# TheJacksonLaboratory/cnn_autoencoder

Hardware: AMD Instinct MI355X
Metric: tiles/sec, compress+decompress round trip of 1024x1024x3 histology tiles (higher is better)
Workload: dtype f32 (f16x3 split MFMA: 3 f16 MFMAs per product, fp32 accumulate)

## Files before the change

### cnn_autoencoder_amd/csrc/cae_api.hip

```cpp
#include "cae_hip.h"
#include "cae_internal.hpp"
#include "cae_kernels.hpp"
#include "cae_kernels_f16.hpp"
#include "cae_launch.hpp"
#include "cae_pack.hpp"

#include <algorithm>
#include <cmath>
#include <cstdio>
#include <cstdlib>
#include <cstring>
#include <string>

namespace cae {

thread_local std::string g_last_error;
thread_local int64_t g_last_ticket = 0;
thread_local int g_force_fp32 = 0;

int fail(int code, const char *fmt, ...) {
    char buf[512];
    va_list ap;
    va_start(ap, fmt);
    vsnprintf(buf, sizeof buf, fmt, ap);
// ... 198 lines not shown

static int pick_slot(int a, int b) {
    for (int k = 1; k <= 3; ++k)
        if (k != a && k != b) return k;
    return 1;
}

static bool stages_need_fp32(const Layer &l) {
    if (round_ct(l.cin) <= 4) return false;
    for (const Layer::Stage &sg : l.stages)
        if (sg.gdn || sg.add_res || sg.post_act) return true;
    return false;
}

static int run_stages(Model *m, const Layer &l, bool synthesis, int n, int ch, int cw, const float *&cur, int &cur_idx,
                      int &cur_planes, hipStream_t st, bool f16 = false, int *flag = nullptr) {
    if (f16 && stages_need_fp32(l)) {
        const int tmp = pick_slot(cur_idx, cur_idx);
        const size_t rows = (size_t)n * cur_planes * ch;
        if (synthesis)
            hipLaunchKernelGGL(c8s_to_c8_kernel<true>, dim3(ew_grid(rows * cw)), dim3(256), 0, st, (const char *)cur,
                               (float *)m->ws[tmp].p, rows, cw);
        else
            hipLaunchKernelGGL(c8s_to_c8_kernel<false>, dim3(ew_grid(rows * cw)), dim3(256), 0, st, (const char *)cur,
                               (float *)m->ws[tmp].p, rows, cw);
        HIP_TRY(hipGetLastError());
        cur = (const float *)m->ws[tmp].p;
        cur_idx = tmp;
        int rc = run_stages(m, l, synthesis, n, ch, cw, cur, cur_idx, cur_planes, st, false, nullptr);
        if (rc) return rc;
        const int back = pick_slot(cur_idx, cur_idx);
        const size_t orows = (size_t)n * cur_planes * ch;
        if (synthesis)
            hipLaunchKernelGGL(c8_to_c8s_kernel<true>, dim3(ew_grid(orows * cw)), dim3(256), 0, st, cur, (char *)m->ws[back].p,
                               orows, cw, flag);
        else
            hipLaunchKernelGGL(c8_to_c8s_kernel<false>, dim3(ew_grid(orows * cw)), dim3(256), 0, st, cur, (char *)m->ws[back].p,
                               orows, cw, flag);
        HIP_TRY(hipGetLastError());
        cur = (const float *)m->ws[back].p;
        cur_idx = back;
        return CAE_OK;
    }
    const float *unit_in = cur;
    const int unit_idx = cur_idx, unit_planes = cur_planes;
    for (const Layer::Stage &sg : l.stages) {
        const int ctin = round_ct(l.cin);
        const int out_idx = pick_slot(unit_idx, cur_idx);
        LayerArgs b = layer_args(m, cur, cur_planes, m->ws[out_idx].p, n, ch, cw, ch, cw, ctin, l.cin, OUT_C8, sg.act,
                                 f16 ? flag : nullptr);
        b.bias = sg.bias.get<float>();
        b.beta = sg.beta.get<float>();
        b.res = sg.add_res ? unit_in : nullptr;
        b.res_planes = unit_planes;
        b.post_act = sg.post_act;
        int rc;
        if (f16) {
            if (!sg.wp16 || (sg.gdn && !sg.gp16)) return fail(CAE_ERR_ARG, "stage uploaded before precision 1 was selected");
            b.wp = sg.wp16.get<float>();
            b.gp = sg.gp16.get<float>();
            rc = launch_conv_s1_f16(m->ks, ctin, synthesis, sg.gdn, l.cin, b, st);
// ... 244 lines not shown
}

static int analysis_impl(cae_model_t *mm, const void *tiles, int fmt, int n, int h, int w, void *latents, bool symbols,
                         float *const *levels, void *stream) {
    Model *m = reinterpret_cast<Model *>(mm);
    if (!m || !tiles || !latents) return fail(CAE_ERR_ARG, "NULL argument");
    if (symbols && m->ent.channels == 0) return fail(CAE_ERR_ARG, "entropy model not set");
    if (n < 1 || h < 2 || w < 2) return fail(CAE_ERR_ARG, "bad tile batch %dx%dx%d", n, h, w);
    if (fmt != CAE_FMT_U8_HWC && fmt != CAE_FMT_F32_NCHW) return fail(CAE_ERR_ARG, "bad pixel format %d", fmt);
    for (auto &l : m->enc)
        if (!l.set) return fail(CAE_ERR_ARG, "analysis layer not set");
    int rc;
    if ((rc = check_reflect_levels(m, h, w))) return rc;
    hipStream_t st = (hipStream_t)stream;
    std::lock_guard<std::mutex> lk(m->mu);
    if ((rc = m->ensure_device()) || (rc = m->order_stream(stream))) return rc;
    const bool f16 = m->f16_usable();
    const bool first_fused = f16 ? (bool)m->enc[0].wp_edge16 : (bool)m->enc[0].wp_edge;
    int64_t ticket = 0;
    g_last_ticket = 0;
    int *flag = f16 ? m->next_flag(&ticket) : m->flags_dev;

    const int p0 = f16 ? 2 * ((m->c_org + 15) / 16) : (m->c_org + 7) / 8;
    auto row_bytes = [&](int cw) { return f16 ? c8s_row_bytes<false>(cw) : (size_t)cw * 32; };
    size_t in_bytes = first_fused ? 0 : (size_t)n * p0 * h * row_bytes(w);
    size_t maxact = 0;
    {
        int ch = h, cw = w;
        for (int i = 0; i < m->L; ++i) {
            if (!m->enc[i].stages.empty())
                maxact = std::max(maxact, (size_t)n * round_ct(m->enc[i].cin) * 4 * ch * row_bytes(cw));
            ch = (ch + 1) / 2;
            cw = (cw + 1) / 2;
            if (i + 1 < m->L) maxact = std::max(maxact, (size_t)n * m->enc[i].ct * 4 * ch * row_bytes(cw));
        }
    }
    const bool u8_wide = f16 && !first_fused && fmt == CAE_FMT_U8_HWC;
    if (u8_wide) maxact = std::max(maxact, (size_t)n * p0 * h * w * 32);
    bool need_third_slot = false;
    for (auto &l : m->enc)
        need_third_slot |= l.stages.size() > 1 || (f16 && (!conv_f16_fits(m->ks, l.ct, l.gdn) || stages_need_fp32(l)));
    if ((rc = m->ensure_ws(0, in_bytes))) return rc;
    if (maxact && ((rc = m->ensure_ws(1, maxact)) || (rc = m->ensure_ws(2, maxact)))) return rc;
    if (maxact && need_third_slot && (rc = m->ensure_ws(3, maxact))) return rc;

    ProfScope prof(m, CAE_ANALYSIS, st);
    prof.begin();
    if (!first_fused) {
        const size_t tot = (size_t)n * p0 * h * w;
        if (f16) {
            if (fmt == CAE_FMT_U8_HWC) {
                hipLaunchKernelGGL(u8hwc_to_c8_kernel, dim3(ew_grid(tot)), dim3(256), 0, st, (const uint8_t *)tiles,
                                   (float *)m->ws[1].p, n, h, w, m->c_org, p0);
                hipLaunchKernelGGL(c8_to_c8s_kernel<false>, dim3(ew_grid(tot)), dim3(256), 0, st, (const float *)m->ws[1].p,
                                   (char *)m->ws[0].p, (size_t)n * p0 * h, w, flag);
            } else {
                hipLaunchKernelGGL(nchw_to_c8s_kernel<false>, dim3(ew_grid(tot)), dim3(256), 0, st,
                                   (const float *)tiles, (char *)m->ws[0].p, n, m->c_org, h, w, p0, flag);
            }
        } else if (fmt == CAE_FMT_U8_HWC) {
            hipLaunchKernelGGL(u8hwc_to_c8_kernel, dim3(ew_grid(tot)), dim3(256), 0, st, (const uint8_t *)tiles,
                               (float *)m->ws[0].p, n, h, w, m->c_org, p0);
        } else {
            hipLaunchKernelGGL(nchw_to_c8_kernel, dim3(ew_grid(tot)), dim3(256), 0, st, (const float *)tiles,
                               (float *)m->ws[0].p, n, m->c_org, h * w, p0);
        }
        HIP_TRY(hipGetLastError());
    }
    prof.end();

    const float *cur = (const float *)m->ws[0].p;
    int cur_planes = p0, ch = h, cw = w;
    int cur_idx = 0;
    for (int i = 0; i < m->L; ++i) {
        const Layer &l = m->enc[i];
        const bool last = i == m->L - 1;
        if (!l.stages.empty() && (rc = run_stages(m, l, false, n, ch, cw, cur, cur_idx, cur_planes, st, f16, flag))) return rc;
        const int out_idx = pick_slot(cur_idx, cur_idx);
        LayerArgs a = layer_args(m, cur, cur_planes, last ? latents : m->ws[out_idx].p, n, ch, cw, (ch + 1) / 2, (cw + 1) / 2,
                                 l.ct, l.cout, last ? (symbols ? OUT_SYM : OUT_NCHW) : OUT_C8, l.act, flag);
        a.wp = l.wp.get<float>();
        a.bias = l.bias.get<float>();
        a.gp = l.gp.get<float>();
        a.beta = l.beta.get<float>();
        if (last && symbols) a.medians = m->medians_dev.get<float>();
        prof.begin();
        if (i == 0 && first_fused) {
            FirstArgs f{tiles, fmt == CAE_FMT_U8_HWC ? 1 : 0, l.cin};
            if (f16) {
                a.wp = l.wp_edge16.get<float>();
                a.gp = l.gp16.get<float>();
                if ((rc = launch_first_f16(m->ks, l.ct, l.gdn, a, f, st))) return rc;
            } else {
                a.wp = l.wp_edge.get<float>();
                if ((rc = launch_first(m->ks, l.ct, l.gdn, a, f, st))) return rc;
            }
        } else if (f16 && conv_f16_fits(m->ks, l.ct, l.gdn) && !(l.gdn && l.ct > 4 && last)) {
            a.wp = l.wp16.get<float>();
            a.gp = l.gp16.get<float>();
            if ((rc = launch_conv_f16(m->ks, l.ct, l.gdn, l.cin, a, st))) return rc;
        } else if (f16) {
            const int tmp_in = pick_slot(cur_idx, out_idx);
            const size_t rows = (size_t)n * cur_planes * ch;
            hipLaunchKernelGGL(c8s_to_c8_kernel<false>, dim3(ew_grid(rows * cw)), dim3(256), 0, st, (const char *)cur,
                               (float *)m->ws[tmp_in].p, rows, cw);
            HIP_TRY(hipGetLastError());
            a.in = (const float *)m->ws[tmp_in].p;
            void *final_out = a.out;
            if (!last) a.out = m->ws[cur_idx == 0 ? pick_slot(tmp_in, out_idx) : cur_idx].p;
            if ((rc = launch_conv(m->ks, l.ct, l.gdn, l.cin, a, st))) return rc;
            if (!last) {
                const size_t orows = (size_t)n * l.ct * 4 * a.OH;
                hipLaunchKernelGGL(c8_to_c8s_kernel<false>, dim3(ew_grid(orows * a.OW)), dim3(256), 0, st, (const float *)a.out,
                                   (char *)final_out, orows, a.OW, flag);
                HIP_TRY(hipGetLastError());
                a.out = final_out;
            }
        } else {
            if ((rc = launch_conv(m->ks, l.ct, l.gdn, l.cin, a, st))) return rc;
        }
        prof.end();
        if (!last && levels && levels[i]) {
            const size_t t2 = (size_t)n * l.cout * a.OH * a.OW;
            if (f16)
                hipLaunchKernelGGL(c8s_to_nchw_kernel<false>, dim3(ew_grid(t2)), dim3(256), 0, st, (const char *)a.out,
                                   levels[i], n, l.cout, a.OH, a.OW, l.ct * 4);
            else
                hipLaunchKernelGGL(c8_to_nchw_kernel, dim3(ew_grid(t2)), dim3(256), 0, st, (const float *)a.out,
                                   levels[i], n, l.cout, a.OH * a.OW, l.ct * 4);
            HIP_TRY(hipGetLastError());
        }
        cur = (const float *)a.out;
        cur_planes = l.ct * 4;
        ch = a.OH;
        cw = a.OW;
        cur_idx = out_idx;
    }
    return CAE_OK;
}

static int synthesis_impl(cae_model_t *mm, const float *latents, const int32_t *symbols, int n, int lh, int lw, void *out,
                          int fmt, float *const *bridges, float *const *colors, void *stream, int scale = 0);

int cae_synthesis(cae_model_t *mm, const float *latents, int n, int lh, int lw, void *out, int fmt,
                  float *const *bridges, void *stream) {
    if (!latents) return fail(CAE_ERR_ARG, "NULL argument");
    return synthesis_impl(mm, latents, nullptr, n, lh, lw, out, fmt, bridges, nullptr, stream);
}
// ... 504 lines not shown
```

### cnn_autoencoder_amd/csrc/cae_kernels.hpp

```cpp
#pragma once
#include <hip/hip_runtime.h>
#include <stdint.h>
#include <type_traits>
#include <utility>

namespace cae {

typedef float f32x16 __attribute__((ext_vector_type(16)));
typedef float f32x4 __attribute__((ext_vector_type(4)));

enum OutFmt { OUT_C8 = 0, OUT_NCHW = 1, OUT_U8HWC = 2, OUT_SYM = 3, OUT_PMAP = 4 };

struct LayerArgs {
    const float *in;
    void *out;
    const float *wp;
    const float *bias;
    const float *gp;
    const float *beta;
    const float *zero;
    int N, H, W, OH, OW;
    int in_planes;
    int cci;
    int out_planes;
    int cout;
    int tiles_x, tiles_y;
    int outfmt;
// ... 2 lines not shown
    int res_planes;
    int post_act;
    const float *medians;
    const void *pm;
    int *flag;
};

__device__ __forceinline__ uint8_t clip_u8(float q) {
    return (uint8_t)__builtin_fmaxf(__builtin_fminf(q, 255.0f), 0.0f);
}
__device__ __forceinline__ int round_sym(float d) {
    return (int)rintf(__builtin_fminf(__builtin_fmaxf(d, -1073741824.0f), 1073741824.0f));
}

template <int N, class F, int... I>
__device__ __forceinline__ void static_for_impl(F &&f, std::integer_sequence<int, I...>) {
    (f(std::integral_constant<int, I>{}), ...);
}
template <int N, class F>
__device__ __forceinline__ void static_for(F &&f) {
    static_for_impl<N>(static_cast<F &&>(f), std::make_integer_sequence<int, N>{});
}

__device__ __forceinline__ int reflect_idx(int i, int n) {
    i = i < 0 ? -i : i;
    i = i >= n ? 2 * n - 2 - i : i;
    i = i < 0 ? 0 : i;
    return i >= n ? n - 1 : i;
}

__device__ __forceinline__ void glds16(const void *gsrc, void *lds_wave_base) {
    __builtin_amdgcn_global_load_lds((const __attribute__((address_space(1))) void *)gsrc,
                                     (__attribute__((address_space(3))) void *)lds_wave_base, 16, 0, 0);
}

__device__ __forceinline__ void wait_vm0() { asm volatile("s_waitcnt vmcnt(0)" ::: "memory"); }

__device__ __forceinline__ constexpr int acc_row(int r) { return (r & 3) + 8 * (r >> 2); }

__device__ __forceinline__ void load_acc_tile(f32x16 &a, const float *vec, int ct, int h) {
#pragma unroll
    for (int g = 0; g < 4; ++g) {
        const f32x4 v = *(const f32x4 *)(vec + 32 * ct + 8 * g + 4 * h);
#pragma unroll
        for (int k = 0; k < 4; ++k) a[4 * g + k] = v[k];
    }
}

template <int CT>
__device__ __forceinline__ void init_acc(f32x16 (&acc)[CT], const float *vec, int h, float fill) {
#pragma unroll
    for (int ct = 0; ct < CT; ++ct) {
        if (vec) {
// ... 1146 lines not shown
```

### cnn_autoencoder_amd/csrc/cae_kernels_f16.hpp

```cpp
#pragma once
#include "cae_kernels.hpp"

namespace cae {

constexpr int F16_ISSUERS = 2;
#define ISSUER(w, NW, NI) ((w) < (NI) ? (w) : -1)

typedef _Float16 f16x8 __attribute__((ext_vector_type(8)));
typedef _Float16 f16x4 __attribute__((ext_vector_type(4)));


__device__ __forceinline__ void split_f16(float v, _Float16 &hi, _Float16 &lo) {
    hi = (_Float16)v;
    lo = (_Float16)(v - (float)hi);
}

typedef unsigned u32x2v __attribute__((ext_vector_type(2)));
__device__ __forceinline__ u32x2v split2_f16(float a, float b) {
    typedef float f32x2 __attribute__((ext_vector_type(2)));
    typedef _Float16 f16x2 __attribute__((ext_vector_type(2)));
    const f32x2 ab = {a, b};
    const unsigned hi = __builtin_bit_cast(unsigned, __builtin_convertvector(ab, f16x2));
    float l0, l1;
    asm("v_fma_mix_f32 %0, %1, -1.0, %2 op_sel_hi:[1,0,0]" : "=v"(l0) : "v"(hi), "v"(a));
// ... 97 lines not shown
                const f16x8 gh = *(const f16x8 *)(gb + ((co * 2 + s) * 2 + 0) * 1024);
                const f16x8 gl = *(const f16x8 *)(gb + ((co * 2 + s) * 2 + 1) * 1024);
#pragma unroll
                for (int pt = 0; pt < PT; ++pt) nrm[pt][co] = mfma3(gh, gl, sh[pt], sl[pt], nrm[pt][co]);
            }
        }
        ++sc;
    }
#pragma unroll
    for (int pt = 0; pt < PT; ++pt) {
#pragma unroll
        for (int ct = 0; ct < CT; ++ct)
#pragma unroll
            for (int r = 0; r < 16; ++r) {
                const float nv = nrm[pt][ct][r];
                if constexpr (INVERSE)
                    y[PT0 + pt][ct][r] *= __builtin_amdgcn_sqrtf(nv) * pisc[pt];
                else
                    y[PT0 + pt][ct][r] *= __builtin_amdgcn_rsqf(nv);
            }
    }
}

template <bool SP>
__host__ __device__ __forceinline__ size_t c8s_row_bytes(int w) {
    return SP ? (size_t)((w + 63) >> 6) * 2048 : (size_t)((w + 31) >> 5) * 1024;
}
template <bool SP>
__host__ __device__ __forceinline__ unsigned c8s_piece(int x) {
    return SP ? (unsigned)(x >> 6) * 2048u + (unsigned)(x & 1) * 1024u + (unsigned)((x & 63) >> 1) * 16u
              : (unsigned)(x >> 5) * 1024u + (unsigned)(x & 31) * 16u;
}

template <int CT, bool SP = false>
__device__ __forceinline__ void store_split_f16(const f32x16 (&acc)[CT], const LayerArgs &p, int n, int oy, int ox, int h,
                                                int ct0 = 0) {
    {
        char *out = (char *)p.out;
        float mx = 0.0f;
#pragma unroll
        for (int ct = 0; ct < CT; ++ct)
#pragma unroll
            for (int r = 0; r < 16; r += 2)
                mx = absmax3(mx, acc[ct][r], acc[ct][r + 1]);
        raise_if_over(mx, p.flag);
        const size_t row_bytes = c8s_row_bytes<SP>(p.OW), plane_bytes = (size_t)p.OH * row_bytes;
        char *dst0 = out + (((size_t)n * p.out_planes + 4 * ct0) * p.OH + oy) * row_bytes + c8s_piece<SP>(ox) + 512 * h;
#pragma unroll
        for (int ct = 0; ct < CT; ++ct)
#pragma unroll
            for (int g = 0; g < 4; ++g) {
                typedef unsigned u32x2 __attribute__((ext_vector_type(2)));
                typedef unsigned u32x4 __attribute__((ext_vector_type(4)));
                u32x2 yh, xl;
                { const u32x2v t_ = split2_f16(acc[ct][4 * g + 0], acc[ct][4 * g + 1]); yh[0] = t_[0]; xl[0] = t_[1]; }
// ... 34 lines not shown

template <int CT, bool SP = false, int EPI = 0>
__device__ __forceinline__ void store_tiles_f16(f32x16 (&acc)[CT], const LayerArgs &p, int n, int oy, int ox,
                                                int h, bool valid) {
    if (!valid) return;
    if (p.outfmt == OUT_C8) {
        if constexpr (EPI & 1) {
            const float slope = p.act == 0 ? 1.0f : (p.act == 1 ? 0.01f : 0.0f);
#pragma unroll
            for (int ct = 0; ct < CT; ++ct)
#pragma unroll
                for (int r = 0; r < 16; ++r) acc[ct][r] = acc[ct][r] > 0.0f ? acc[ct][r] : slope * acc[ct][r];
        }
        if constexpr (EPI & 2) {
            if (p.res) add_residual_f16<CT, SP>(acc, p, n, oy, ox, h);
        }
        store_split_f16<CT, SP>(acc, p, n, oy, ox, h);
    } else {
        store_tiles<CT, false>(acc, p, n, oy, ox, h, valid);
    }
}

constexpr int CONV_F16_NW = 8;
template <int KS, int CT, bool GDN, int S = 2, bool SP = false, bool ZP = false, bool RES = false>
__global__ void __launch_bounds__(CONV_F16_NW * 64, 1) conv_s2_f16_kernel(const LayerArgs p) {
    constexpr int NW = CONV_F16_NW, PT = 8 / NW;
    constexpr int PAD = KS / 2;
    constexpr int TX = 16, TY = 16;
    constexpr int WH = S * TX + KS - S;
    constexpr int PLANE_PIECES = TY * WH;
    constexpr int HALO_PIECES = 4 * PLANE_PIECES;
    constexpr int HALO_INSTR = (HALO_PIECES + 63) / 64;
    constexpr int W_INSTR = KS * CT * 2;
    constexpr int W_BYTES = W_INSTR * 1024;
    constexpr int G_BYTES = GDN ? CT * 4096 : 0;
    constexpr int CONV_STAGE = W_BYTES + HALO_INSTR * 1024;
    constexpr int STAGE_BYTES = CONV_STAGE > G_BYTES ? CONV_STAGE : G_BYTES;
    constexpr int NI = NW / F16_ISSUERS > 0 ? NW / F16_ISSUERS : 1;
    constexpr int MAXP = (HALO_INSTR + NI - 1) / NI;
    extern __shared__ __attribute__((aligned(16))) char smem[];

    const int lane = threadIdx.x & 63;
    const int wave = __builtin_amdgcn_readfirstlane(threadIdx.x >> 6);
    const int h = lane >> 5, m = lane & 31;

    int bid = xcd_tile_order(blockIdx.x, gridDim.x);
    const int tx = bid % p.tiles_x;
    bid /= p.tiles_x;
    const int ty = bid % p.tiles_y;
    const int n = bid / p.tiles_y;
    const int oy0 = ty * TY, ox0 = tx * TX;

    const size_t plane_bytes = (size_t)p.H * c8s_row_bytes<SP>(p.W);
    const char *in_n = (const char *)p.in + (size_t)n * p.in_planes * plane_bytes;
    unsigned hoff[MAXP][KS];
#pragma unroll
    for (int i = 0; i < MAXP; ++i) {
        int pc = (ISSUER(wave, NW, NI) + i * NI) * 64 + lane;
        pc = pc < HALO_PIECES ? pc : HALO_PIECES - 1;
        const int plhl = pc / PLANE_PIECES;
        const int rem = pc - plhl * PLANE_PIECES;
        const int r = rem / WH, x = rem - r * WH;
        const int xi = S * ox0 - PAD + x;
// ... 430 lines not shown
                const int t0 = 4 * s + half, t1 = 4 * s + 2 + half;
                const int o0 = t0 < KS * KS ? ((t0 / KS) * WH + (t0 % KS)) * 16 : -1;
                const int o1 = t1 < KS * KS ? ((t1 / KS) * WH + (t1 % KS)) * 16 : -1;
                f32x4 v0 = {0.f, 0.f, 0.f, 0.f}, v1 = {0.f, 0.f, 0.f, 0.f};
                if (o0 >= 0) v0 = *(const f32x4 *)(hb + o0);
                if (o1 >= 0) v1 = *(const f32x4 *)(hb + o1);
                const f32x4 v = h ? v1 : v0;
                { const u32x2v t_ = split2_f16(v[0], v[1]); bhw[2 * half] = t_[0]; blw[2 * half] = t_[1]; }
                { const u32x2v t_ = split2_f16(v[2], v[3]); bhw[2 * half + 1] = t_[0]; blw[2 * half + 1] = t_[1]; }
            }
            const f16x8 bh = __builtin_bit_cast(f16x8, bhw), bl = __builtin_bit_cast(f16x8, blw);
#pragma unroll
            for (int ct = 0; ct < CT; ++ct) {
                const f16x8 ah = *(const f16x8 *)(wb + ((s * CT + ct) * 2 + 0) * 1024);
                const f16x8 al = *(const f16x8 *)(wb + ((s * CT + ct) * 2 + 1) * 1024);
                acc[ct] = mfma3(ah, al, bh, bl, acc[ct]);
            }
        }
        __builtin_amdgcn_wave_barrier();
        if (has_next) commit();
        __builtin_amdgcn_wave_barrier();
        if constexpr (GDN) gdn_resident_pipe_f16<CT, false>(acc, gbuf, beta_lds, lane);
        const int oy = ty * TY + 2 * wave + (m >> 4), ox = tx * TX + (m & 15);
        store_tiles_f16<CT, false, !GDN>(acc, p, n, oy, ox, h, oy < p.OH && ox < p.OW);
    }
    if constexpr (!U8)
        if (bad) *p.flag = 1;
}

__host__ __device__ __forceinline__ size_t pmap_record(int n, int OH, int OW, int oy, int ox) {
    return ((((size_t)n * OH + oy) * 2 + (ox & 1)) * (OW >> 1) + (ox >> 1)) * 32;
}

template <int CT, int LDS_JT>
__device__ __forceinline__ void store_pmap_f16(const f32x16 (&y)[CT], const LayerArgs &p, char *tbuf, int n, int oy, int par,
                                               int j0, int lane, bool row_valid, const char *pm_lds) {
    const int h = lane >> 5, m = lane & 31;
    f32x16 pm;
#pragma unroll
    for (int r = 0; r < 16; ++r) pm[r] = 0.0f;
    float mx = 0.0f;
#pragma unroll
    for (int jt = 0; jt < CT; ++jt)
#pragma unroll
        for (int s = 0; s < 2; ++s) {
            const char *ab = (jt < LDS_JT ? pm_lds : (const char *)p.pm) + lane * 16;
            u32x4v hw, lw;
// ... 574 lines not shown
```

### cnn_autoencoder_amd/csrc/cae_launch.hpp

```cpp
#pragma once
#include <hip/hip_runtime.h>

#include <map>
#include <mutex>
#include <utility>

#include "cae_hip.h"
#include "cae_internal.hpp"

#define HIP_TRY(expr)                                                                             \
    do {                                                                                          \
        hipError_t e_ = (expr);                                                                   \
        if (e_ != hipSuccess) return ::cae::fail(CAE_ERR_HIP, "%s: %s", #expr, hipGetErrorString(e_));  \
    } while (0)

#define CAE_TRY(expr)                          \
    do {                                       \
        const int rc_ = (expr);                \
        if (rc_ != CAE_OK) return rc_;         \
    } while (0)

namespace cae {
inline std::mutex &launch_mutex() {
    static std::mutex mu;
// ... 17 lines not shown
    int dev = 0;
    HIP_TRY(hipGetDevice(&dev));
    static std::map<int, int> known;
    std::lock_guard<std::mutex> lock(launch_mutex());
    auto it = known.find(dev);
    if (it == known.end()) {
        int n = 0;
        HIP_TRY(hipDeviceGetAttribute(&n, hipDeviceAttributeMultiprocessorCount, dev));
        it = known.emplace(dev, n).first;
    }
    cus = it->second;
    return CAE_OK;
}

template <class Args>
Args with_launch_facts(const Args &a, int w, int h, int tx, int ty, int cci) {
    Args b = a;
    b.tiles_x = (w + tx - 1) / tx;
    b.tiles_y = (h + ty - 1) / ty;
    b.cci = cci;
    return b;
}

struct LayerArgs;
struct FirstArgs;
int launch_conv(int ks, int ct, bool gdn, int cin, const LayerArgs &a, hipStream_t st);
int launch_conv_s1(int ks, int ct, bool zeropad, bool gdn, int cin, const LayerArgs &a, hipStream_t st);
int launch_deconv(int ks, int ct, bool gdn, int cin, const LayerArgs &a, hipStream_t st);
int launch_gdn(int ct, bool inverse, const LayerArgs &a, hipStream_t st);
int launch_first(int ks, int ct, bool gdn, const LayerArgs &a, const FirstArgs &f, hipStream_t st);
int launch_last(int ks, int cin, const LayerArgs &a, hipStream_t st);
int launch_conv_f16(int ks, int ct, bool gdn, int cin, const LayerArgs &a, hipStream_t st);
int launch_deconv_f16(int ks, int ct, bool gdn, int cin, const LayerArgs &a, hipStream_t st);
int launch_conv_s1_f16(int ks, int ct, bool synthesis, bool gdn, int cin, const LayerArgs &a, hipStream_t st);
int launch_color_f16(int ks, int cin, const LayerArgs &a, hipStream_t st);
bool conv_f16_fits(int ks, int ct, bool gdn);
bool last_f16_fits(int ks, int cin);
int launch_color_small(int ks, bool split, const void *in, int in_planes, int cin, const float *w, const float *bias,
                       int n, int h, int w_px, int cout, void *out, int outfmt, int *flag, hipStream_t st);
int launch_nchw_to_u8hwc(const float *in, void *out, int n, int c, size_t hw, hipStream_t st);
int launch_first_f16(int ks, int ct, bool gdn, const LayerArgs &a, const FirstArgs &f, hipStream_t st);
int launch_last_f16(int ks, int cin, const LayerArgs &a, hipStream_t st);
int launch_gdn_f16(int ct, bool inverse, const LayerArgs &a, hipStream_t st);
}
```

### cnn_autoencoder_amd/csrc/cae_launch_conv_f16.hip

```cpp
#include "cae_hip.h"
#include "cae_internal.hpp"
#include "cae_launch.hpp"
#include "cae_kernels_f16.hpp"
namespace cae {
constexpr int LDS_LIMIT = 160 * 1024;

constexpr int conv_f16_lds(int ks, int ct, bool gdn, int wh) {
    const int halo_instr = (4 * 16 * wh + 63) / 64;
    const int conv_stage = ks * ct * 2 * 1024 + halo_instr * 1024;
    const int g_bytes = gdn ? ct * 4096 : 0;
    return 2 * (conv_stage > g_bytes ? conv_stage : g_bytes);
}
constexpr int conv_f16_halo_width(int ks, int stride) { return stride * 16 + ks - stride; }

bool conv_f16_fits(int ks, int ct, bool gdn) {
    if (gdn && ct > 4) gdn = false;
    return conv_f16_lds(ks, ct, gdn, conv_f16_halo_width(ks, 2)) <= LDS_LIMIT;
}

static LayerArgs conv_f16_facts(const LayerArgs &a, int cin) {
    return with_launch_facts(a, a.OW, a.OH, 16, 16, (cin + 15) / 16);
}

template <int KS, int CT, bool GDN>
static int launch_conv_f16_t(int cin, const LayerArgs &args, hipStream_t st) {
    constexpr int NW = CONV_F16_NW;
    constexpr int LDS = conv_f16_lds(KS, CT, GDN, conv_f16_halo_width(KS, 2));
    if constexpr (LDS > LDS_LIMIT) {
        return fail(CAE_ERR_UNSUPPORTED, "f16x3: this kernel_size/channel combination exceeds the LDS; use fp32");
    } else {
        auto kern = conv_s2_f16_kernel<KS, CT, GDN>;
        CAE_TRY(ensure_lds((const void *)kern, LDS));
        const LayerArgs a = conv_f16_facts(args, cin);
        const unsigned grid = (unsigned)((size_t)a.N * a.tiles_x * a.tiles_y);
        hipLaunchKernelGGL(kern, dim3(grid), dim3(NW * 64), LDS, st, a);
        HIP_TRY(hipGetLastError());
        return CAE_OK;
    }
}

#define DISPATCH_F16(FN, KS_)                                                               \
    switch (ct) {                                                                          \
        case 1: return gdn ? FN<KS_, 1, true>(cin, a, st) : FN<KS_, 1, false>(cin, a, st); \
        case 2: return gdn ? FN<KS_, 2, true>(cin, a, st) : FN<KS_, 2, false>(cin, a, st); \
        case 4: return gdn ? FN<KS_, 4, true>(cin, a, st) : FN<KS_, 4, false>(cin, a, st); \
        case 6: {  \
            const int rc6 = FN<KS_, 6, false>(cin, a, st);                                 \
            return rc6 || !gdn ? rc6 : launch_gdn_f16(6, false, a, st);                    \
        }                                                                                  \
        default: return fail(CAE_ERR_UNSUPPORTED, "unsupported channel tiles %d", ct);      \
    }

template <int KS, int CT, bool GDN, bool SYN, bool ZP>
static int launch_conv_s1_f16_t(int cin, const LayerArgs &args, hipStream_t st) {
    constexpr int NW = CONV_F16_NW;
    constexpr int LDS = conv_f16_lds(KS, CT, GDN, conv_f16_halo_width(KS, 1));
    if constexpr (LDS > LDS_LIMIT) {
        return fail(CAE_ERR_UNSUPPORTED, "f16x3: this kernel_size/channel combination exceeds the LDS; use fp32");
    } else {
        auto kern = conv_s2_f16_kernel<KS, CT, GDN, 1, SYN, ZP, (CT <= 4)>;
        CAE_TRY(ensure_lds((const void *)kern, LDS));
        const LayerArgs a = conv_f16_facts(args, cin);
        const unsigned grid = (unsigned)((size_t)a.N * a.tiles_x * a.tiles_y);
        hipLaunchKernelGGL(kern, dim3(grid), dim3(NW * 64), LDS, st, a);
        HIP_TRY(hipGetLastError());
        return CAE_OK;
    }
}

int launch_conv_s1_f16(int ks, int ct, bool synthesis, bool gdn, int cin, const LayerArgs &a, hipStream_t st) {
    if ((gdn || a.res || a.post_act) && ct > 4)
        return fail(CAE_ERR_UNSUPPORTED, "f16x3: GDN / residual stages wider than 128 channels run on the fp32 path");
#define S1_SIDE(KS_, CT_, GDN_) \
    return synthesis ? launch_conv_s1_f16_t<KS_, CT_, GDN_, true, true>(cin, a, st) \
                     : launch_conv_s1_f16_t<KS_, CT_, GDN_, false, false>(cin, a, st)
#define S1_CASE(KS_)                                                                   \
    switch (ct) {                                                                      \
        case 1: if (gdn) { S1_SIDE(KS_, 1, true); } else { S1_SIDE(KS_, 1, false); }   \
        case 2: if (gdn) { S1_SIDE(KS_, 2, true); } else { S1_SIDE(KS_, 2, false); }   \
        case 4: if (gdn) { S1_SIDE(KS_, 4, true); } else { S1_SIDE(KS_, 4, false); }   \
        case 6: S1_SIDE(KS_, 6, false);                                                \
        default: return fail(CAE_ERR_UNSUPPORTED, "unsupported channel tiles %d", ct);  \
    }
    if (ks == 3) { S1_CASE(3) }
    if (ks == 5) { S1_CASE(5) }
#undef S1_CASE
#undef S1_SIDE
    return fail(CAE_ERR_UNSUPPORTED, "kernel_size %d not supported (3 or 5)", ks);
}

int launch_color_f16(int ks, int cin, const LayerArgs &a, hipStream_t st) {
    if (ks == 3) return launch_conv_s1_f16_t<3, 1, false, true, false>(cin, a, st);
    if (ks == 5) return launch_conv_s1_f16_t<5, 1, false, true, false>(cin, a, st);
    return fail(CAE_ERR_UNSUPPORTED, "kernel_size %d not supported (3 or 5)", ks);
}

int launch_conv_f16(int ks, int ct, bool gdn, int cin, const LayerArgs &a, hipStream_t st) {
    if (ks == 3) { DISPATCH_F16(launch_conv_f16_t, 3) }
// ... 6 lines not shown
```

### cnn_autoencoder_amd/csrc/cae_launch_edge_f16.hip

```cpp
#include <algorithm>

#include "cae_hip.h"
#include "cae_internal.hpp"
#include "cae_launch.hpp"
#include "cae_kernels_f16.hpp"
namespace cae {
template <int KS, int CT, bool GDN>
static int launch_first_f16_t(const LayerArgs &a, const FirstArgs &f, hipStream_t st) {
    using G = FirstGeomF16<KS, CT, GDN>;
    constexpr int LDS = G::LDS_BYTES;
    if constexpr (LDS > 160 * 1024) {
        return fail(CAE_ERR_UNSUPPORTED, "f16x3: first-layer operands exceed the LDS for this shape; use fp32");
    } else {
        auto kern_u8 = conv_first_f16_kernel<KS, CT, GDN, true>;
        auto kern_f32 = conv_first_f16_kernel<KS, CT, GDN, false>;
        int n_cu = 0;
        CAE_TRY(ensure_lds((const void *)kern_u8, LDS));
        CAE_TRY(ensure_lds((const void *)kern_f32, LDS));
        CAE_TRY(device_cus(n_cu));
        const LayerArgs b = with_launch_facts(a, a.OW, a.OH, G::TX, G::TY, (f.cin + 7) / 8);
        const size_t total = (size_t)b.N * b.tiles_x * b.tiles_y;
        if (total > 0x7fffffff) return fail(CAE_ERR_ARG, "batch too large");
        const unsigned grid = (unsigned)std::min<size_t>(total, (size_t)std::max(n_cu, 1));
        hipLaunchKernelGGL(f.in_is_u8 ? kern_u8 : kern_f32, dim3(grid), dim3(G::NW * 64), LDS, st, b, f);
// ... 3 lines not shown
}

int launch_first_f16(int ks, int ct, bool gdn, const LayerArgs &a, const FirstArgs &f, hipStream_t st) {
#define FIRST_F16(KS_)                                                                                       \
    switch (ct) {                                                                                            \
        case 1: return gdn ? launch_first_f16_t<KS_, 1, true>(a, f, st) : launch_first_f16_t<KS_, 1, false>(a, f, st); \
        case 2: return gdn ? launch_first_f16_t<KS_, 2, true>(a, f, st) : launch_first_f16_t<KS_, 2, false>(a, f, st); \
        case 4: return gdn ? launch_first_f16_t<KS_, 4, true>(a, f, st) : launch_first_f16_t<KS_, 4, false>(a, f, st); \
        case 6: {                                                                                            \
            const int rc6 = launch_first_f16_t<KS_, 6, false>(a, f, st);                                     \
            return rc6 || !gdn ? rc6 : launch_gdn_f16(6, false, a, st);                                      \
        }                                                                                                    \
        default: return fail(CAE_ERR_UNSUPPORTED, "unsupported channel tiles %d", ct);                       \
    }
    if (ks == 3) { FIRST_F16(3) }
    if (ks == 5) { FIRST_F16(5) }
    return fail(CAE_ERR_UNSUPPORTED, "kernel_size %d not supported (3 or 5)", ks);
}

template <int CT, bool INVERSE>
static int launch_gdn_f16_t(const LayerArgs &a, hipStream_t st) {
    constexpr int LDS = CT * CT * 4096 + CT * 32 * 4;
    static_assert(LDS <= 160 * 1024, "packed gamma must fit the LDS");
    auto kern = gdn_f16_kernel<CT, INVERSE, INVERSE>;
    int n_cu = 0;
    CAE_TRY(ensure_lds((const void *)kern, LDS));
    CAE_TRY(device_cus(n_cu));
    const size_t groups = c8s_row_bytes<INVERSE>(a.OW) / 1024;
    const size_t total = (size_t)a.N * a.OH * groups;
    if (total > 0x7fffffff) return fail(CAE_ERR_ARG, "batch too large");
    const unsigned grid = (unsigned)std::min<size_t>((total + 3) / 4, (size_t)std::max(n_cu, 1));
    hipLaunchKernelGGL(kern, dim3(grid), dim3(256), LDS, st, a);
    HIP_TRY(hipGetLastError());
    return CAE_OK;
}

int launch_gdn_f16(int ct, bool inverse, const LayerArgs &a, hipStream_t st) {
    if (a.outfmt != OUT_C8) return fail(CAE_ERR_UNSUPPORTED, "f16x3: stand-alone GDN needs split rows as output");
    if (ct == 6) return inverse ? launch_gdn_f16_t<6, true>(a, st) : launch_gdn_f16_t<6, false>(a, st);
    return fail(CAE_ERR_UNSUPPORTED, "stand-alone GDN is built for 192-channel layers (channel tiles %d)", ct);
}

using LastF16K3 = LastGeomF16<3, 8, 3>;
using LastF16K5 = LastGeomF16<5, 4, 2>;

bool last_f16_fits(int ks, int cin) {
    const int nq = (cin + 31) / 32;
    return (ks == 3 ? LastF16K3::lds_bytes(nq) : LastF16K5::lds_bytes(nq)) <= 160 * 1024;
}

template <int KS, class G>
// ... 25 lines not shown
```

Before: 4040.

## Switch analysis f16 rows to parity-split layout with a row-tiled strided conv kernel

Analysis-side split-f16 activations now use the parity-split (SP) row layout everywhere, and the stride-2 convolution gets a dedicated kernel that tiles 8 output rows by 32 columns. That kernel loads even and odd input columns as aligned 1 KiB pieces plus a few stray edge pieces directly into LDS. The aim is to avoid gathering strided pixels from a 2D halo, so each LDS stage carries less wasted halo and loads stay contiguous. The risk is that every producer and consumer must agree on the new layout: conversions, GDN, stride-1 layers and the first layer's store all change together.

```diff
diff --git a/cnn_autoencoder_amd/csrc/cae_api.hip b/cnn_autoencoder_amd/csrc/cae_api.hip
--- a/cnn_autoencoder_amd/csrc/cae_api.hip
+++ b/cnn_autoencoder_amd/csrc/cae_api.hip
@@ -244,7 +244,7 @@
             hipLaunchKernelGGL(c8s_to_c8_kernel<true>, dim3(ew_grid(rows * cw)), dim3(256), 0, st, (const char *)cur,
                                (float *)m->ws[tmp].p, rows, cw);
         else
-            hipLaunchKernelGGL(c8s_to_c8_kernel<false>, dim3(ew_grid(rows * cw)), dim3(256), 0, st, (const char *)cur,
+            hipLaunchKernelGGL(c8s_to_c8_kernel<F16_ROWS_SP>, dim3(ew_grid(rows * cw)), dim3(256), 0, st, (const char *)cur,
                                (float *)m->ws[tmp].p, rows, cw);
         HIP_TRY(hipGetLastError());
         cur = (const float *)m->ws[tmp].p;
@@ -257,8 +257,8 @@
             hipLaunchKernelGGL(c8_to_c8s_kernel<true>, dim3(ew_grid(orows * cw)), dim3(256), 0, st, cur, (char *)m->ws[back].p,
                                orows, cw, flag);
         else
-            hipLaunchKernelGGL(c8_to_c8s_kernel<false>, dim3(ew_grid(orows * cw)), dim3(256), 0, st, cur, (char *)m->ws[back].p,
-                               orows, cw, flag);
+            hipLaunchKernelGGL(c8_to_c8s_kernel<F16_ROWS_SP>, dim3(ew_grid(orows * cw)), dim3(256), 0, st, cur,
+                               (char *)m->ws[back].p, orows, cw, flag);
         HIP_TRY(hipGetLastError());
         cur = (const float *)m->ws[back].p;
         cur_idx = back;
@@ -549,7 +549,7 @@
     int *flag = f16 ? m->next_flag(&ticket) : m->flags_dev;
 
     const int p0 = f16 ? 2 * ((m->c_org + 15) / 16) : (m->c_org + 7) / 8;
-    auto row_bytes = [&](int cw) { return f16 ? c8s_row_bytes<false>(cw) : (size_t)cw * 32; };
+    auto row_bytes = [&](int cw) { return f16 ? c8s_row_bytes<F16_ROWS_SP>(cw) : (size_t)cw * 32; };
     size_t in_bytes = first_fused ? 0 : (size_t)n * p0 * h * row_bytes(w);
     size_t maxact = 0;
     {
@@ -579,10 +579,10 @@
             if (fmt == CAE_FMT_U8_HWC) {
                 hipLaunchKernelGGL(u8hwc_to_c8_kernel, dim3(ew_grid(tot)), dim3(256), 0, st, (const uint8_t *)tiles,
                                    (float *)m->ws[1].p, n, h, w, m->c_org, p0);
-                hipLaunchKernelGGL(c8_to_c8s_kernel<false>, dim3(ew_grid(tot)), dim3(256), 0, st, (const float *)m->ws[1].p,
-                                   (char *)m->ws[0].p, (size_t)n * p0 * h, w, flag);
+                hipLaunchKernelGGL(c8_to_c8s_kernel<F16_ROWS_SP>, dim3(ew_grid(tot)), dim3(256), 0, st,
+                                   (const float *)m->ws[1].p, (char *)m->ws[0].p, (size_t)n * p0 * h, w, flag);
             } else {
-                hipLaunchKernelGGL(nchw_to_c8s_kernel<false>, dim3(ew_grid(tot)), dim3(256), 0, st,
+                hipLaunchKernelGGL(nchw_to_c8s_kernel<F16_ROWS_SP>, dim3(ew_grid(tot)), dim3(256), 0, st,
                                    (const float *)tiles, (char *)m->ws[0].p, n, m->c_org, h, w, p0, flag);
             }
         } else if (fmt == CAE_FMT_U8_HWC) {
@@ -629,7 +629,7 @@
         } else if (f16) {
             const int tmp_in = pick_slot(cur_idx, out_idx);
             const size_t rows = (size_t)n * cur_planes * ch;
-            hipLaunchKernelGGL(c8s_to_c8_kernel<false>, dim3(ew_grid(rows * cw)), dim3(256), 0, st, (const char *)cur,
+            hipLaunchKernelGGL(c8s_to_c8_kernel<F16_ROWS_SP>, dim3(ew_grid(rows * cw)), dim3(256), 0, st, (const char *)cur,
                                (float *)m->ws[tmp_in].p, rows, cw);
             HIP_TRY(hipGetLastError());
             a.in = (const float *)m->ws[tmp_in].p;
@@ -638,8 +638,8 @@
             if ((rc = launch_conv(m->ks, l.ct, l.gdn, l.cin, a, st))) return rc;
             if (!last) {
                 const size_t orows = (size_t)n * l.ct * 4 * a.OH;
-                hipLaunchKernelGGL(c8_to_c8s_kernel<false>, dim3(ew_grid(orows * a.OW)), dim3(256), 0, st, (const float *)a.out,
-                                   (char *)final_out, orows, a.OW, flag);
+                hipLaunchKernelGGL(c8_to_c8s_kernel<F16_ROWS_SP>, dim3(ew_grid(orows * a.OW)), dim3(256), 0, st,
+                                   (const float *)a.out, (char *)final_out, orows, a.OW, flag);
                 HIP_TRY(hipGetLastError());
                 a.out = final_out;
             }
@@ -650,7 +650,7 @@
         if (!last && levels && levels[i]) {
             const size_t t2 = (size_t)n * l.cout * a.OH * a.OW;
             if (f16)
-                hipLaunchKernelGGL(c8s_to_nchw_kernel<false>, dim3(ew_grid(t2)), dim3(256), 0, st, (const char *)a.out,
+                hipLaunchKernelGGL(c8s_to_nchw_kernel<F16_ROWS_SP>, dim3(ew_grid(t2)), dim3(256), 0, st, (const char *)a.out,
                                    levels[i], n, l.cout, a.OH, a.OW, l.ct * 4);
             else
                 hipLaunchKernelGGL(c8_to_nchw_kernel, dim3(ew_grid(t2)), dim3(256), 0, st, (const float *)a.out,
diff --git a/cnn_autoencoder_amd/csrc/cae_kernels.hpp b/cnn_autoencoder_amd/csrc/cae_kernels.hpp
--- a/cnn_autoencoder_amd/csrc/cae_kernels.hpp
+++ b/cnn_autoencoder_amd/csrc/cae_kernels.hpp
@@ -3,6 +3,8 @@
 #include <stdint.h>
 #include <type_traits>
 #include <utility>
+
+#include "cae_rows_f16.hpp"
 
 namespace cae {
 
@@ -51,13 +53,6 @@
     static_for_impl<N>(static_cast<F &&>(f), std::make_integer_sequence<int, N>{});
 }
 
-__device__ __forceinline__ int reflect_idx(int i, int n) {
-    i = i < 0 ? -i : i;
-    i = i >= n ? 2 * n - 2 - i : i;
-    i = i < 0 ? 0 : i;
-    return i >= n ? n - 1 : i;
-}
-
 __device__ __forceinline__ void glds16(const void *gsrc, void *lds_wave_base) {
     __builtin_amdgcn_global_load_lds((const __attribute__((address_space(1))) void *)gsrc,
                                      (__attribute__((address_space(3))) void *)lds_wave_base, 16, 0, 0);
diff --git a/cnn_autoencoder_amd/csrc/cae_kernels_f16.hpp b/cnn_autoencoder_amd/csrc/cae_kernels_f16.hpp
--- a/cnn_autoencoder_amd/csrc/cae_kernels_f16.hpp
+++ b/cnn_autoencoder_amd/csrc/cae_kernels_f16.hpp
@@ -143,15 +143,6 @@
     }
 }
 
-template <bool SP>
-__host__ __device__ __forceinline__ size_t c8s_row_bytes(int w) {
-    return SP ? (size_t)((w + 63) >> 6) * 2048 : (size_t)((w + 31) >> 5) * 1024;
-}
-template <bool SP>
-__host__ __device__ __forceinline__ unsigned c8s_piece(int x) {
-    return SP ? (unsigned)(x >> 6) * 2048u + (unsigned)(x & 1) * 1024u + (unsigned)((x & 63) >> 1) * 16u
-              : (unsigned)(x >> 5) * 1024u + (unsigned)(x & 31) * 16u;
-}
 
 template <int CT, bool SP = false>
 __device__ __forceinline__ void store_split_f16(const f32x16 (&acc)[CT], const LayerArgs &p, int n, int oy, int ox, int h,
@@ -232,6 +223,137 @@
 }
 
 constexpr int CONV_F16_NW = 8;
+
+template <int KS, int CT, bool GDN>
+struct ConvGeomF16 {
+    static constexpr int NW = CONV_F16_NW, ROWS = NW, TX = 32;
+    static constexpr int PAD = KS / 2;
+    static constexpr int NSTRAY = KS - 2;
+    static constexpr int AL_INSTR = 4 * 2 * ROWS * 32 / 64;
+    static constexpr int AL_BYTES = AL_INSTR * 1024;
+    static constexpr int STRAY_PIECES = NSTRAY * 4 * ROWS;
+    static constexpr int STRAY_INSTR = (STRAY_PIECES + 63) / 64;
+    static constexpr int HALO_INSTR = AL_INSTR + STRAY_INSTR;
+    static constexpr int W_INSTR = KS * CT * 2;
+    static constexpr int W_BYTES = W_INSTR * 1024;
+    static constexpr int G_BYTES = GDN ? CT * 4096 : 0;
+    static constexpr int CONV_STAGE = W_BYTES + HALO_INSTR * 1024;
+    static constexpr int STAGE_BYTES = CONV_STAGE > G_BYTES ? CONV_STAGE : G_BYTES;
+    static constexpr int LDS_BYTES = 2 * STAGE_BYTES;
+    static constexpr int NI = NW / F16_ISSUERS > 0 ? NW / F16_ISSUERS : 1;
+    static constexpr int AL_PER = AL_INSTR / NI;
+    static_assert(ROWS == 8 && NI == 4 && STRAY_INSTR <= NI, "issuer waves each cover one row pair of every aligned image");
+    static constexpr int B_HL = 2 * ROWS * 32 * 16, B_HL_STRAY = ROWS * 16;
+};
+
+template <int KS, int CT, bool GDN>
+__device__ __forceinline__ void conv_s2_rows_f16(const LayerArgs &p, char *smem) {
+    using G = ConvGeomF16<KS, CT, GDN>;
+    constexpr int NW = G::NW, NI = G::NI, PAD = G::PAD, ROWS = G::ROWS;
+    constexpr int W_BYTES = G::W_BYTES, W_INSTR = G::W_INSTR, STAGE_BYTES = G::STAGE_BYTES;
+
+    const int lane = threadIdx.x & 63;
+    const int wave = __builtin_amdgcn_readfirstlane(threadIdx.x >> 6);
+    const int h = lane >> 5, m = lane & 31;
+
+    int bid = xcd_tile_order(blockIdx.x, gridDim.x);
+    const int tx = bid % p.tiles_x;
+    bid /= p.tiles_x;
+    const int ty = bid % p.tiles_y;
+    const int n = bid / p.tiles_y;
+    const int oy0 = ty * ROWS, ox0 = tx * G::TX;
+
+    const size_t row_bytes = c8s_row_bytes<true>(p.W), plane_bytes = (size_t)p.H * row_bytes;
+    const char *in_n = (const char *)p.in + (size_t)n * p.in_planes * plane_bytes;
+    const int iw0 = ISSUER(wave, NW, NI) < 0 ? 0 : ISSUER(wave, NW, NI);
+    unsigned xoff[2], yoff[KS], soff, syoff[KS];
+    {
+#pragma unroll
+        for (int par = 0; par < 2; ++par) xoff[par] = c8s_piece<true>(conv_rows_aligned_px(ox0, m, par, p.W));
+        int pc = iw0 * 64 + lane;
+        pc = pc < G::STRAY_PIECES ? pc : G::STRAY_PIECES - 1;
+        const int s = pc / (4 * ROWS), pl = (pc / (2 * ROWS)) & 1, hl = (pc / ROWS) & 1, rs = pc % ROWS;
+        soff = (unsigned)pl * (unsigned)plane_bytes + (unsigned)hl * 512u + c8s_piece<true>(conv_rows_stray_px(ox0, s, PAD, p.W));
+#pragma unroll
+        for (int ky = 0; ky < KS; ++ky) {
+            yoff[ky] = (unsigned)conv_rows_input_row(oy0 + 2 * iw0 + h, ky, PAD, p.H) * (unsigned)row_bytes;
+            syoff[ky] = (unsigned)conv_rows_input_row(oy0 + rs, ky, PAD, p.H) * (unsigned)row_bytes;
+        }
+    }
+    const unsigned woff = (unsigned)lane * 16u;
+
+    auto issue_stage = [&](int q, auto ky_tag, char *buf) {
+        constexpr int ky = decltype(ky_tag)::value;
+        if (ISSUER(wave, NW, NI) < 0) return;
+        const int iw = ISSUER(wave, NW, NI);
+        const char *wsrc = (const char *)p.wp + (size_t)(q * KS + ky) * W_BYTES;
+#pragma unroll
+        for (int i = 0; i < (W_INSTR + NI - 1) / NI; ++i) {
+            const int j = iw + i * NI;
+            if (j < W_INSTR) glds16(wsrc + j * 1024 + woff, buf + j * 1024);
+        }
+        const char *planes = in_n + (size_t)(2 * q) * plane_bytes;
+#pragma unroll
+        for (int i = 0; i < G::AL_PER; ++i) {
+            const char *src = planes + (size_t)(i >> 2) * plane_bytes + ((i >> 1) & 1) * 512 + xoff[i & 1] + yoff[ky];
+            glds16(src, buf + W_BYTES + (iw + i * NI) * 1024);
+        }
+        if (iw < G::STRAY_INSTR) glds16(planes + soff + syoff[ky], buf + W_BYTES + (G::AL_INSTR + iw) * 1024);
+    };
+
+    f32x16 acc[1][CT];
+    init_acc<CT>(acc[0], p.bias, h, 0.0f);
+
+    int b_off[KS], b_hl[KS];
+#pragma unroll
+    for (int kx = 0; kx < KS; ++kx) {
+        const ConvRowsTap t = conv_rows_tap(kx, PAD, m);
+        b_off[kx] = W_BYTES + (t.stray >= 0 ? G::AL_BYTES + (((t.stray * 2 + h) * 2) * ROWS + wave) * 16
+                                            : ((((h * 2) * 2 + t.par) * ROWS + wave) * 32 + t.col) * 16);
+        b_hl[kx] = t.stray >= 0 ? G::B_HL_STRAY : G::B_HL;
+    }
+    int sc = 0;
+
+    issue_stage(0, std::integral_constant<int, 0>{}, smem);
+    for (int q = 0; q < p.cci; ++q) {
+        static_for<KS>([&](auto ky_tag) {
+            constexpr int ky = decltype(ky_tag)::value;
+            wait_vm0();
+            __syncthreads();
+            char *cur = smem + (sc & 1) * STAGE_BYTES;
+            char *nxt = smem + ((sc + 1) & 1) * STAGE_BYTES;
+            if constexpr (ky + 1 < KS) {
+                issue_stage(q, std::integral_constant<int, ky + 1>{}, nxt);
+            } else {
+                if (q + 1 < p.cci) {
+                    issue_stage(q + 1, std::integral_constant<int, 0>{}, nxt);
+                } else if (GDN) {
+                    issue_gamma0<CT, NW>(p, nxt, wave, lane);
+                }
+            }
+            const char *wb = cur + lane * 16;
+#pragma unroll
+            for (int kx = 0; kx < KS; ++kx) {
+                const f16x8 bh = *(const f16x8 *)(cur + b_off[kx]);
+                const f16x8 bl = *(const f16x8 *)(cur + b_off[kx] + b_hl[kx]);
+#pragma unroll
+                for (int ct = 0; ct < CT; ++ct) {
+                    const f16x8 ah = *(const f16x8 *)(wb + ((kx * CT + ct) * 2 + 0) * 1024);
+                    const f16x8 al = *(const f16x8 *)(wb + ((kx * CT + ct) * 2 + 1) * 1024);
+                    acc[0][ct] = mfma3(ah, al, bh, bl, acc[0][ct]);
+                }
+            }
+            ++sc;
+        });
+    }
+
+    if constexpr (GDN) {
+        gdn_stages_f16<CT, 1, NW, false, STAGE_BYTES>(acc, p, smem, sc, wave, lane, [](char *) {});
+    }
+    const int oy = oy0 + wave, ox = ox0 + m;
+    store_tiles_f16<CT, true, GDN ? 0 : 1>(acc[0], p, n, oy, ox, h, oy < p.OH && ox < p.OW);
+}
+
 template <int KS, int CT, bool GDN, int S = 2, bool SP = false, bool ZP = false, bool RES = false>
 __global__ void __launch_bounds__(CONV_F16_NW * 64, 1) conv_s2_f16_kernel(const LayerArgs p) {
     constexpr int NW = CONV_F16_NW, PT = 8 / NW;
@@ -249,6 +371,11 @@
     constexpr int NI = NW / F16_ISSUERS > 0 ? NW / F16_ISSUERS : 1;
     constexpr int MAXP = (HALO_INSTR + NI - 1) / NI;
     extern __shared__ __attribute__((aligned(16))) char smem[];
+    if constexpr (S == 2) {
+        static_assert(SP && !ZP && !RES, "the strided layer reads and writes C8SP rows, reflect padding");
+        conv_s2_rows_f16<KS, CT, GDN>(p, smem);
+        return;
+    }
 
     const int lane = threadIdx.x & 63;
     const int wave = __builtin_amdgcn_readfirstlane(threadIdx.x >> 6);
@@ -725,7 +852,7 @@
         __builtin_amdgcn_wave_barrier();
         if constexpr (GDN) gdn_resident_pipe_f16<CT, false>(acc, gbuf, beta_lds, lane);
         const int oy = ty * TY + 2 * wave + (m >> 4), ox = tx * TX + (m & 15);
-        store_tiles_f16<CT, false, !GDN>(acc, p, n, oy, ox, h, oy < p.OH && ox < p.OW);
+        store_tiles_f16<CT, true, !GDN>(acc, p, n, oy, ox, h, oy < p.OH && ox < p.OW);
     }
     if constexpr (!U8)
         if (bad) *p.flag = 1;
diff --git a/cnn_autoencoder_amd/csrc/cae_launch.hpp b/cnn_autoencoder_amd/csrc/cae_launch.hpp
--- a/cnn_autoencoder_amd/csrc/cae_launch.hpp
+++ b/cnn_autoencoder_amd/csrc/cae_launch.hpp
@@ -63,6 +63,8 @@
     return b;
 }
 
+constexpr bool F16_ROWS_SP = true;
+
 struct LayerArgs;
 struct FirstArgs;
 int launch_conv(int ks, int ct, bool gdn, int cin, const LayerArgs &a, hipStream_t st);
diff --git a/cnn_autoencoder_amd/csrc/cae_launch_conv_f16.hip b/cnn_autoencoder_amd/csrc/cae_launch_conv_f16.hip
--- a/cnn_autoencoder_amd/csrc/cae_launch_conv_f16.hip
+++ b/cnn_autoencoder_amd/csrc/cae_launch_conv_f16.hip
@@ -5,33 +5,36 @@
 namespace cae {
 constexpr int LDS_LIMIT = 160 * 1024;
 
-constexpr int conv_f16_lds(int ks, int ct, bool gdn, int wh) {
-    const int halo_instr = (4 * 16 * wh + 63) / 64;
+constexpr int conv_f16_lds(int ks, int ct, bool gdn, int stride) {
+    const int halo_instr = stride == 2 ? 4 * 2 * 8 * 32 / 64 + ((ks - 2) * 4 * 8 + 63) / 64 : (4 * 16 * (16 + ks - 1) + 63) / 64;
     const int conv_stage = ks * ct * 2 * 1024 + halo_instr * 1024;
     const int g_bytes = gdn ? ct * 4096 : 0;
     return 2 * (conv_stage > g_bytes ? conv_stage : g_bytes);
 }
-constexpr int conv_f16_halo_width(int ks, int stride) { return stride * 16 + ks - stride; }
+static_assert(conv_f16_lds(3, 6, false, 2) <= LDS_LIMIT && conv_f16_lds(5, 4, true, 2) <= LDS_LIMIT,
+              "k = 3 up to 192 channels and k = 5 up to 128 channels run on the split-f16 kernel");
 
 bool conv_f16_fits(int ks, int ct, bool gdn) {
     if (gdn && ct > 4) gdn = false;
-    return conv_f16_lds(ks, ct, gdn, conv_f16_halo_width(ks, 2)) <= LDS_LIMIT;
+    return conv_f16_lds(ks, ct, gdn, 2) <= LDS_LIMIT;
 }
 
-static LayerArgs conv_f16_facts(const LayerArgs &a, int cin) {
-    return with_launch_facts(a, a.OW, a.OH, 16, 16, (cin + 15) / 16);
+static LayerArgs conv_f16_facts(const LayerArgs &a, int cin, int stride) {
+    return stride == 2 ? with_launch_facts(a, a.OW, a.OH, 32, 8, (cin + 15) / 16)
+                       : with_launch_facts(a, a.OW, a.OH, 16, 16, (cin + 15) / 16);
 }
 
 template <int KS, int CT, bool GDN>
 static int launch_conv_f16_t(int cin, const LayerArgs &args, hipStream_t st) {
     constexpr int NW = CONV_F16_NW;
-    constexpr int LDS = conv_f16_lds(KS, CT, GDN, conv_f16_halo_width(KS, 2));
+    constexpr int LDS = conv_f16_lds(KS, CT, GDN, 2);
     if constexpr (LDS > LDS_LIMIT) {
         return fail(CAE_ERR_UNSUPPORTED, "f16x3: this kernel_size/channel combination exceeds the LDS; use fp32");
     } else {
-        auto kern = conv_s2_f16_kernel<KS, CT, GDN>;
+        static_assert(LDS == ConvGeomF16<KS, CT, GDN>::LDS_BYTES, "conv_f16_lds restates the kernel's stage layout");
+        auto kern = conv_s2_f16_kernel<KS, CT, GDN, 2, F16_ROWS_SP>;
         CAE_TRY(ensure_lds((const void *)kern, LDS));
-        const LayerArgs a = conv_f16_facts(args, cin);
+        const LayerArgs a = conv_f16_facts(args, cin, 2);
         const unsigned grid = (unsigned)((size_t)a.N * a.tiles_x * a.tiles_y);
         hipLaunchKernelGGL(kern, dim3(grid), dim3(NW * 64), LDS, st, a);
         HIP_TRY(hipGetLastError());
@@ -51,16 +54,16 @@
         default: return fail(CAE_ERR_UNSUPPORTED, "unsupported channel tiles %d", ct);      \
     }
 
-template <int KS, int CT, bool GDN, bool SYN, bool ZP>
+template <int KS, int CT, bool GDN, bool SP, bool ZP>
 static int launch_conv_s1_f16_t(int cin, const LayerArgs &args, hipStream_t st) {
     constexpr int NW = CONV_F16_NW;
-    constexpr int LDS = conv_f16_lds(KS, CT, GDN, conv_f16_halo_width(KS, 1));
+    constexpr int LDS = conv_f16_lds(KS, CT, GDN, 1);
     if constexpr (LDS > LDS_LIMIT) {
         return fail(CAE_ERR_UNSUPPORTED, "f16x3: this kernel_size/channel combination exceeds the LDS; use fp32");
     } else {
-        auto kern = conv_s2_f16_kernel<KS, CT, GDN, 1, SYN, ZP, (CT <= 4)>;
+        auto kern = conv_s2_f16_kernel<KS, CT, GDN, 1, SP, ZP, (CT <= 4)>;
         CAE_TRY(ensure_lds((const void *)kern, LDS));
-        const LayerArgs a = conv_f16_facts(args, cin);
+        const LayerArgs a = conv_f16_facts(args, cin, 1);
         const unsigned grid = (unsigned)((size_t)a.N * a.tiles_x * a.tiles_y);
         hipLaunchKernelGGL(kern, dim3(grid), dim3(NW * 64), LDS, st, a);
         HIP_TRY(hipGetLastError());
@@ -73,7 +76,7 @@
         return fail(CAE_ERR_UNSUPPORTED, "f16x3: GDN / residual stages wider than 128 channels run on the fp32 path");
 #define S1_SIDE(KS_, CT_, GDN_) \
     return synthesis ? launch_conv_s1_f16_t<KS_, CT_, GDN_, true, true>(cin, a, st) \
-                     : launch_conv_s1_f16_t<KS_, CT_, GDN_, false, false>(cin, a, st)
+                     : launch_conv_s1_f16_t<KS_, CT_, GDN_, F16_ROWS_SP, false>(cin, a, st)
 #define S1_CASE(KS_)                                                                   \
     switch (ct) {                                                                      \
         case 1: if (gdn) { S1_SIDE(KS_, 1, true); } else { S1_SIDE(KS_, 1, false); }   \
diff --git a/cnn_autoencoder_amd/csrc/cae_launch_edge_f16.hip b/cnn_autoencoder_amd/csrc/cae_launch_edge_f16.hip
--- a/cnn_autoencoder_amd/csrc/cae_launch_edge_f16.hip
+++ b/cnn_autoencoder_amd/csrc/cae_launch_edge_f16.hip
@@ -49,11 +49,12 @@
 static int launch_gdn_f16_t(const LayerArgs &a, hipStream_t st) {
     constexpr int LDS = CT * CT * 4096 + CT * 32 * 4;
     static_assert(LDS <= 160 * 1024, "packed gamma must fit the LDS");
-    auto kern = gdn_f16_kernel<CT, INVERSE, INVERSE>;
+    constexpr bool SP = INVERSE || F16_ROWS_SP;
+    auto kern = gdn_f16_kernel<CT, INVERSE, SP>;
     int n_cu = 0;
     CAE_TRY(ensure_lds((const void *)kern, LDS));
     CAE_TRY(device_cus(n_cu));
-    const size_t groups = c8s_row_bytes<INVERSE>(a.OW) / 1024;
+    const size_t groups = c8s_row_bytes<SP>(a.OW) / 1024;
     const size_t total = (size_t)a.N * a.OH * groups;
     if (total > 0x7fffffff) return fail(CAE_ERR_ARG, "batch too large");
     const unsigned grid = (unsigned)std::min<size_t>((total + 3) / 4, (size_t)std::max(n_cu, 1));
diff --git a/cnn_autoencoder_amd/csrc/cae_rows_f16.hpp b/cnn_autoencoder_amd/csrc/cae_rows_f16.hpp
--- /dev/null
+++ b/cnn_autoencoder_amd/csrc/cae_rows_f16.hpp
@@ -0,0 +1,42 @@
+#pragma once
+#include <stddef.h>
+
+#ifdef __HIP__
+#define CAE_HD __host__ __device__ __forceinline__
+#else
+#define CAE_HD inline
+#endif
+
+namespace cae {
+
+CAE_HD int reflect_idx(int i, int n) {
+    i = i < 0 ? -i : i;
+    i = i >= n ? 2 * n - 2 - i : i;
+    i = i < 0 ? 0 : i;
+    return i >= n ? n - 1 : i;
+}
+
+template <bool SP>
+CAE_HD size_t c8s_row_bytes(int w) {
+    return SP ? (size_t)((w + 63) >> 6) * 2048 : (size_t)((w + 31) >> 5) * 1024;
+}
+template <bool SP>
+CAE_HD unsigned c8s_piece(int x) {
+    return SP ? (unsigned)(x >> 6) * 2048u + (unsigned)(x & 1) * 1024u + (unsigned)((x & 63) >> 1) * 16u
+              : (unsigned)(x >> 5) * 1024u + (unsigned)(x & 31) * 16u;
+}
+
+CAE_HD int conv_rows_aligned_px(int ox0, int m, int par, int w) { return reflect_idx(2 * (ox0 + m) + par, w); }
+CAE_HD int conv_rows_stray_px(int ox0, int s, int pad, int w) {
+    return reflect_idx(2 * ox0 + (s < pad ? s - pad : 64 + s - pad), w);
+}
+CAE_HD int conv_rows_input_row(int oy, int ky, int pad, int h) { return reflect_idx(2 * oy + ky - pad, h); }
+struct ConvRowsTap {
+    int par, col, stray;
+};
+CAE_HD ConvRowsTap conv_rows_tap(int kx, int pad, int m) {
+    const int d = kx - pad, col = m + (d >> 1);
+    return ConvRowsTap{d & 1, col, col < 0 ? pad + d : (col > 31 ? pad + d - 2 : -1)};
+}
+
+}
```

Result: no change. 4077 (median of 3 runs) (+0.9%).
